# antonbaumann/MIMO-Unet

Measured on AMD Instinct MI355X. Metric: train images/sec at 256x256, S=2, fbc=30, higher is better.
Workload: dtype f32 (split into 16-bit hi/lo pairs on the MFMA; weight gradient: activation as one fp16 value); 1 GPU; cfg3: SEN12TP-shape synthetic 2->1 ch, 256x256, S=2, fbc=30, laplace_nll, batch 32 global; global_batch=32, per_gpu_batch=32, scaling=strong, labels=U[0,1) (SURVEY 8d); same batch every step, parallelism=dp1, world_size=1, weak_per_gpu_batch=32, strong_global_batch=32, optimizer=adam(lr=1e-3) fused, inputs=resident in HBM

## Files before the change

### include/mimo_hip.h

```cpp
#ifndef MIMO_HIP_H
#define MIMO_HIP_H

#include <stddef.h>
#include <stdint.h>

#ifdef __cplusplus
extern "C" {
#endif
#if defined(__GNUC__) || defined(__clang__)
#pragma GCC visibility push(default)
#endif

typedef struct mimo_plan mimo_plan;
typedef void* mimo_stream;

enum mimo_status {
  MIMO_OK = 0,
  MIMO_ERR_INVALID = -1,
  MIMO_ERR_HIP = -2,
  MIMO_ERR_STATE = -3
};

enum mimo_precision {
  MIMO_PREC_FP32 = 0,
// ... 214 lines not shown
  const float* z;
  int32_t ldz;
  const float *scale, *shift, *mean, *invstd;
  const float* mask;
  float* dz;
  float *dgamma, *dbeta, *dbias;
  float *c1, *c2;
  float *head_dw, *head_db;
  float* absmax;
  int32_t absmax_capacity;
  int32_t* absmax_n;
  int32_t* status;
} mimo_op_bn_relu_backward_args;
int mimo_op_bn_relu_backward(const mimo_op_bn_relu_backward_args* args, mimo_stream stream);

typedef struct mimo_op_head_backward_args {
  const float* a;
  int32_t lda;
  const float* w;
  int32_t c, c_p, co, n, subnetworks, s;
  int64_t hw;
  const float *out, *dout, *dloss, *label, *mask;
  const int64_t* perm;
  int32_t loss_kind;
  float eps_min, eps_max;
  const float *in_scale, *in_shift;
  int32_t precision;
  float *da, *dw, *db;
} mimo_op_head_backward_args;
int mimo_op_head_backward(const mimo_op_head_backward_args* args, mimo_stream stream);
// ... 109 lines not shown
```

### mimo_unet_amd/_lib.py

```python
from __future__ import annotations

import ctypes as C
import os

import torch

_HERE = os.path.dirname(os.path.abspath(__file__))
LIB_PATH = os.environ.get("MIMO_HIP_LIB") or os.path.join(_HERE, "libmimo_hip.so")


class MimoHipError(RuntimeError):
    pass


class MimoConfig(C.Structure):
    _fields_ = [
        ("in_channels", C.c_int32), ("out_channels", C.c_int32), ("num_subnetworks", C.c_int32),
        ("filter_base_count", C.c_int32), ("batch", C.c_int32), ("height", C.c_int32), ("width", C.c_int32),
        ("encoder_dropout_rate", C.c_float), ("core_dropout_rate", C.c_float), ("decoder_dropout_rate", C.c_float),
        ("bn_eps", C.c_float), ("bn_momentum", C.c_float), ("loss_kind", C.c_int32),
        ("eps_min", C.c_float), ("eps_max", C.c_float), ("device", C.c_int32), ("precision", C.c_int32),
        ("inference_only", C.c_int32), ("center_dropout_rate", C.c_float), ("final_dropout_rate", C.c_float),
        ("norm_kind", C.c_int32), ("act_kind", C.c_int32), ("up_kind", C.c_int32),
    ]
# ... 145 lines not shown
    "mimo_eval_accumulate": (C.c_int, [_P, _P, _P, _P, _P, _I, _I, _I, _I, _L, _I, _F, _F, _P, _I, _P, _P, _P]),
    "mimo_eval_select": (C.c_int, [_P, _L, _P, _I, _P, _P]),
    "mimo_eval_interval_sums": (C.c_int, [_P, _L, _I, _I, _P, _P, _P]),
    "mimo_eval_accumulate_sources": (C.c_int, [_P, _P, _P, _P, _P, _I, _I, _I, _I, _L, _I, _F, _F, _P, _I, _P, _P, _P, _P]),
    "mimo_eval_select_by": (C.c_int, [_P, _I, _L, _P, _I, _P, _P]),
    "mimo_eval_interval_sums_by": (C.c_int, [_P, _I, _P, _I, _L, _I, _I, _P, _P, _P]),
    "mimo_op_conv3x3_forward": (C.c_int, [_P, _P, _P, _P, _P, _I, _I, _I, _I, _I, _I, _I, _I, _P]),
    "mimo_op_conv3x3_dgrad": (C.c_int, [_P, _P, _P, _I, _I, _I, _I, _I, _I, _I, _I, _P]),
    "mimo_op_conv3x3_wgrad": (C.c_int, [_P, _P, _P, _P, _I, _I, _I, _I, _I, _I, _I, _I, _P]),
    "mimo_op_maxpool2x2": (C.c_int, [_P, _P, _I, _I, _I, _I, _P]),
    "mimo_op_upsample_cat": (C.c_int, [_P, _P, _P, _I, _I, _I, _I, _I, _I, _I, _P]),
    "mimo_op_fold_slice": (C.c_int, [_P, _I, _I, _P, _I, _I, _I, _I, _I, _I, _I, _P]),
    "mimo_op_pool_backward": (C.c_int, [_P, _I, _I, _P, _I, _P, _I, _P, _I, _I, _I, _I, _I, _I, _I, _P]),
    "mimo_op_up_backward": (C.c_int, [_P, _I, _I, _P, _I, _I, _I, _I, _I, _I, _I, _I, _I, _P]),
    "mimo_op_bn_relu_backward": (C.c_int, [C.POINTER(BnReluBackwardArgs), _P]),
    "mimo_op_head_backward": (C.c_int, [C.POINTER(HeadBackwardArgs), _P]),
    "mimo_op_bn_stats": (C.c_int, [C.POINTER(BnStatsArgs), _P]),
    "mimo_op_bn_relu_forward": (C.c_int, [C.POINTER(BnReluForwardArgs), _P]),
    "mimo_op_maxpool2x2_ex": (C.c_int, [_P, _I, _P, _I, _I, _I, _I, _I, _I, _P]),
    "mimo_op_upsample_cat_ex": (C.c_int, [_P, _I, _P, _I, _P, _P, _P, _I, _I, _I, _I, _I, _I, _I, _I, _P]),
    "mimo_op_head_forward": (C.c_int, [C.POINTER(HeadForwardArgs), _P]),
    "mimo_op_loss_forward": (C.c_int, [_P, _P, _P, _P, _I, _I, _I, _I, _I, _F, _F, _P, _P]),
    "mimo_op_pack_input": (C.c_int, [_P, _L, _L, _L, _P, _I, _I, _I, _I, _I, _P, _I, _P]),
    "mimo_op_unpack_dx": (C.c_int, [_P, _I, _I, _I, _I, _I, _I, _I, _I, _P, _P]),
    "mimo_op_fold_image_grad": (C.c_int, [_P, _I, _I, _I, _I, _I, _P, _I, _P]),
    "mimo_op_fold_image_grad_mc": (C.c_int, [_P, _I, _I, _I, _I, _I, _I, _P, _I, _P]),
    "mimo_monitor_grid_shape": (C.c_int, [C.c_int, C.c_int, C.c_int, C.c_int, C.c_int, C.POINTER(C.c_int), C.POINTER(C.c_int)]),
    "mimo_monitor_scratch_bytes": (C.c_size_t, [C.c_int]),
    "mimo_monitor_grids": (C.c_int, [C.POINTER(MonitorPanel), C.c_int, _P, _P, _P]),
    "mimo_dataset_gather": (C.c_int, [C.POINTER(GatherField), C.c_int, _P, _P, _L, _I, _I, _I, _P]),
# ... 37 lines not shown
```

### mimo_unet_amd/csrc/conv_thin.hip

```cpp
#include <algorithm>

#include "common.h"

namespace mimo {

namespace {

__device__ __forceinline__ float4 ld4f(const float* p) { return *reinterpret_cast<const float4*>(p); }
__device__ __forceinline__ void st4f(float* p, float4 v) { *reinterpret_cast<float4*>(p) = v; }

struct ThinMap {
  int q, pl, QB, PPI;
  bool active;
};
__device__ __forceinline__ ThinMap thin_map(int Cv) {
  ThinMap t;
  t.QB = Cv;
  t.PPI = 256 / Cv;
  t.q = threadIdx.x % Cv;
  t.pl = threadIdx.x / Cv;
  t.active = t.pl < t.PPI;
  return t;
}

// ... 241 lines not shown
      __syncthreads();
      if (t.pl == 0) {
        float4 s = red[t.q];
        for (int j = 1; j < t.PPI; ++j) {
          const float4 o = red[j * t.QB + t.q];
          s.x += o.x;
          s.y += o.y;
          s.z += o.z;
          s.w += o.w;
        }
        st4f(out + ((size_t)tap * CIN + ci) * 4 * Cv + c0, s);
      }
    }
}

__global__ __launch_bounds__(256) void wgrad_thin_reduce_kernel(const float* __restrict__ partial, int blocks, int cin, int Cp,
                                                                int cout, float* __restrict__ dw) {
  __shared__ double red[256];
  const int tc = blockIdx.x;
  const int tap = tc / cin, ci = tc - tap * cin;
  const int lanes = 256 / Cp;
  const int c = threadIdx.x % Cp, l = threadIdx.x / Cp;
  double s = 0.0;
  if (l < lanes)
    for (int b = l; b < blocks; b += lanes) s += (double)partial[((size_t)b * 9 * cin + tc) * Cp + c];
  red[threadIdx.x] = s;
  __syncthreads();
  if (l == 0 && c < cout) {
    for (int j = 1; j < lanes; ++j) s += red[j * Cp + c];
    dw[((size_t)c * cin + ci) * 9 + tap] = (float)s;
// ... 7 lines not shown
bool thin_enabled() { return thin_level() != 0; }

}

constexpr int kThinBlocks = 2048;

template <typename K>
static int resident_blocks(K kernel) {
  int dev = 0, cus = 256, per_cu = 2;
  if (hipGetDevice(&dev) == hipSuccess) {
    (void)hipDeviceGetAttribute(&cus, hipDeviceAttributeMultiprocessorCount, dev);
    if (hipOccupancyMaxActiveBlocksPerMultiprocessor(&per_cu, kernel, 256, 0) != hipSuccess || per_cu < 1) per_cu = 2;
  }
  return std::min(cus * per_cu, kThinBlocks);
}
struct ThinCaps {
  int fwd[4], wg[4];
};
static const ThinCaps& thin_caps() {
  static const ThinCaps c = {{resident_blocks(conv3x3_thin_fwd_kernel<1>), resident_blocks(conv3x3_thin_fwd_kernel<2>),
                              resident_blocks(conv3x3_thin_fwd_kernel<3>), resident_blocks(conv3x3_thin_fwd_kernel<4>)},
                             {resident_blocks(wgrad_thin_kernel<1>), resident_blocks(wgrad_thin_kernel<2>),
                              resident_blocks(wgrad_thin_kernel<3>), resident_blocks(wgrad_thin_kernel<4>)}};
  return c;
}

int conv3x3_thin_ok(int cin, int cout_p) {
  if (!(thin_enabled() && sched::thin_geometry_ok(cin, cout_p))) return 0;
  (void)thin_caps();
  return 1;
}

int conv3x3_thin_launch(const ConvLaunch& a, int cin, int* rows, hipStream_t stream) {
  if (!conv3x3_thin_ok(cin, a.cout_store) || a.off != 1 || a.Hi != a.Ho || a.Wi != a.Wo || a.Hi < 2 || a.Wi < 2 || a.cin_p < cin ||
      a.ldx % 4 != 0 || a.ldy % 4 != 0 || (int64_t)a.N * a.Hi * a.Wi > INT32_MAX) {
    set_error("conv3x3_thin: bad geometry cin=%d cout=%d H=%d W=%d", cin, a.cout_store, a.Hi, a.Wi);
    return MIMO_ERR_INVALID;
  }
// ... 28 lines not shown
  const int Cv = cout_p / 4;
  const int tilesY = (H + kTH - 1) / kTH, tilesX = (W + kTW - 1) / kTW, numTiles = N * tilesY * tilesX;
  const int blocks = std::min(numTiles, thin_caps().wg[cin - 1]);
  switch (cin) {
    case 1: hipLaunchKernelGGL(wgrad_thin_kernel<1>, dim3(blocks), dim3(256), 0, stream, x, ldx, dz, lddz, N, H, W, Cv, tilesY, tilesX, numTiles, partial); break;
    case 2: hipLaunchKernelGGL(wgrad_thin_kernel<2>, dim3(blocks), dim3(256), 0, stream, x, ldx, dz, lddz, N, H, W, Cv, tilesY, tilesX, numTiles, partial); break;
    case 3: hipLaunchKernelGGL(wgrad_thin_kernel<3>, dim3(blocks), dim3(256), 0, stream, x, ldx, dz, lddz, N, H, W, Cv, tilesY, tilesX, numTiles, partial); break;
    default: hipLaunchKernelGGL(wgrad_thin_kernel<4>, dim3(blocks), dim3(256), 0, stream, x, ldx, dz, lddz, N, H, W, Cv, tilesY, tilesX, numTiles, partial); break;
  }
  MIMO_KERNEL_CHECK();
  hipLaunchKernelGGL(wgrad_thin_reduce_kernel, dim3(9 * cin), dim3(256), 0, stream, partial, blocks, cin, cout_p, cout, dw);
  MIMO_KERNEL_CHECK();
  return MIMO_OK;
}

}
```

### mimo_unet_amd/csrc/elementwise.h

```cpp
#pragma once
#include "common.h"

namespace mimo {

constexpr int kMaxChunks = 64;
constexpr int kEwMaxBlocks = 1024;
constexpr int kBnReduceMaxBlocks = 2048;
constexpr int kMaxHeadOut = 8;

int rowsum_launch(const float* partial, int rows, int cols, double* sums, int* chunks, hipStream_t s);
constexpr int kColsumMaxRows = 2048;
constexpr int kStatusFwdStats = 1, kStatusBwdStats = 2, kStatusLogits = 4;
int colsum_vec_launch(const float* partial, int rows, int cols, int C, float* out, hipStream_t st);
int bn_fwd_stats_launch(const float* partial, int rows, int cout_pad, int C, int Cp, int64_t count, const float* gamma,
                        const float* beta, float* running_mean, float* running_var, float momentum, float eps, float* mean,
                        float* invstd, float* scale, float* shift, int* status, hipStream_t st);
int bn_bwd_stats_launch(const float* partial, int rows, int C, int Cp, int64_t count, int training, float* c1, float* c2,
                        float* dgamma, float* dbeta, float* dbias_zero, int* status, hipStream_t st);
int head_bwd_stats_launch(const float* partial, int rows, int C, int Cp, int Co, float* dw, float* db, hipStream_t st);

int pack_input_launch(const float* x, int64_t stride_n, int64_t stride_s, const int64_t* perm, int s, int N, int C,
                      int H, int W, float* out, int cp, hipStream_t st);
int unpack_dx_launch(const void* dxpad, int dt, int ldp, int N, int S, int s, int C, int H, int W, float* dx, hipStream_t st);

// ... 89 lines not shown
  }
};
int bnrelu_bwd_reduce_launch(const BnReluLayer& L, const GradSrc& src, const float* mask, float* partial, int* rows,
                             hipStream_t st);
struct BnBwdApplyOut {
  const float *c1, *c2;
  void* dz;
  int split_out;
  float* partial;
  int* rows;
  float* absmax;
  int* absmax_n;
  hipEvent_t done;
};
int bn_bwd_apply_launch(const BnReluLayer& L, const GradSrc& src, const float* mask, const BnBwdApplyOut& out, hipStream_t st);
int split_pairs_launch(const float* src, float* dst, int64_t P, int Cp, hipStream_t st, float* absmax = nullptr,
                       int* absmax_n = nullptr);

int head_fwd_launch(const void* a, int dt, int lda, const float* w, const float* bias, int C, int Co, int N, int S, int s,
                    int HW, float* out, hipStream_t st, int* status = nullptr, const float* in_scale = nullptr,
                    const float* in_shift = nullptr);
int loss_fwd_launch(const float* out, const float* label, const float* mask, const int64_t* perm, int N, int S,
                    int Co, int HW, int kind, float eps_min, float eps_max, float* partial, int* blocks,
                    hipStream_t st);
int loss_finalize_launch(const float* partial, int S, int blocks, double count, float* loss_out, hipStream_t st);
int head_bwd_launch(const void* a, int dt, int lda, const float* w, int C, int Cp, int Co, int N, int S, int s, int HW,
                    const float* out, const float* dout, const float* dloss, const float* label, const float* mask,
                    const int64_t* perm, int kind, float eps_min, float eps_max, void* da, float* partial,
                    int* rows, hipStream_t st, const float* in_scale = nullptr, const float* in_shift = nullptr);

// ... 2 lines not shown
```

### mimo_unet_amd/csrc/ew_bn_bwd.hip

```cpp
#include "ew_device.h"

namespace mimo {

__device__ __forceinline__ float route_max(float g, float v00, float v01, float v10, float v11, int self) {
  int arg = 0;
  float m = v00;
  if (v01 > m) { m = v01; arg = 1; }
  if (v10 > m) { m = v10; arg = 2; }
  if (v11 > m) { m = v11; arg = 3; }
  return arg == self ? g : 0.f;
}

template <typename T>
__global__ void pool_bwd_kernel(const T* __restrict__ dxpad, int ldp, int choff, const T* __restrict__ a,
                                int lda, T* __restrict__ da, int ldda, int N, int H, int W, int Cv, int accumulate,
                                const T* __restrict__ skip, int ldsk) {
  const PQ t = pixquad(Cv);
  if (!t.active) return;
  const int Hp = H / 2, Wp = W / 2;
  const int P = N * Hp * Wp;
  PixIter it = pix_iter(t.p, t.pstep, Hp, Wp);
  for (int p = t.p; p < P; p += t.pstep, pix_next(it, Hp, Wp)) {
    const int n = it.n, py = it.y, px = it.x;
    const float4 g = fold_read(dxpad, ldp, n, py, px, Hp, Wp, choff + 4 * t.q);
// ... 182 lines not shown
    st4(dst, v);
  }
}


int up_bwd_launch(const void* dxpad, int dt, int ldp, int choff, void* da, int ldda, int N, int H, int W, int h, int w,
                  int Cp, int accumulate, hipStream_t st) {
  const int Cv = Cp / 4;
  const int padT = (H - 2 * h) / 2, padL = (W - 2 * w) / 2;
  MIMO_ST_DISPATCH(dt, T, hipLaunchKernelGGL(up_bwd_kernel<T>, pq_grid(Cv, (int64_t)N * h * w, kBlocksUpBwd), dim3(256), 0, st,
                                             (const T*)dxpad, ldp, choff, (T*)da, ldda, N, H, W, h, w, padT, padL, Cv, accumulate));
  MIMO_KERNEL_CHECK();
  return MIMO_OK;
}

__device__ __forceinline__ float4 relu_gate4(float4 g, float4 v, float4 sc, float4 sh) {
  g.x = fmaf(v.x, sc.x, sh.x) > 0.f ? g.x : 0.f;
  g.y = fmaf(v.y, sc.y, sh.y) > 0.f ? g.y : 0.f;
  g.z = fmaf(v.z, sc.z, sh.z) > 0.f ? g.z : 0.f;
  g.w = fmaf(v.w, sc.w, sh.w) > 0.f ? g.w : 0.f;
  return g;
}

template <typename TZ, typename TA>
__device__ __forceinline__ int pool_cell4(const GradSrc& s, const TZ* z, int ldz, int n, int cy, int cx, int H, int W, int q,
                                          float4 sc, float4 sh, bool masked, float4 m, float4 zz[4], float4 g[4]) {
  const int Hp = H / 2, Wp = W / 2, y0 = 2 * cy, x0 = 2 * cx;
  const bool win = cy < Hp && cx < Wp;
  const int valid = win ? 15 : ((1 | (x0 + 1 < W ? 2 : 0)) | (y0 + 1 < H ? (4 | (x0 + 1 < W ? 8 : 0)) : 0));
  const TZ* zs = z + (((size_t)n * H + y0) * W + x0) * ldz + 4 * q;
#pragma unroll
  for (int j = 0; j < 4; ++j) zz[j] = (valid >> j) & 1 ? ld4(zs + ((size_t)(j >> 1) * W + (j & 1)) * ldz) : f4zero();
  float4 gp = f4zero();
  if (win) gp = fold_read((const TA*)s.dxpad, s.ldp, n, cy, cx, Hp, Wp, s.choff + 4 * q);
#pragma unroll
  for (int j = 0; j < 4; ++j)
    g[j] = (s.skip && ((valid >> j) & 1)) ? fold_read((const TA*)s.skip, s.ldsk, n, y0 + (j >> 1), x0 + (j & 1), H, W, s.skoff + 4 * q)
                                           : f4zero();
// ... 6 lines not shown
      g[j].z = route_max(gp.z, act(zz[0].z, sc.z, sh.z, m.z), act(zz[1].z, sc.z, sh.z, m.z), act(zz[2].z, sc.z, sh.z, m.z), act(zz[3].z, sc.z, sh.z, m.z), j) + g[j].z;
      g[j].w = route_max(gp.w, act(zz[0].w, sc.w, sh.w, m.w), act(zz[1].w, sc.w, sh.w, m.w), act(zz[2].w, sc.w, sh.w, m.w), act(zz[3].w, sc.w, sh.w, m.w), j) + g[j].w;
    }
  }
#pragma unroll
  for (int j = 0; j < 4; ++j) {
    if (masked) {
      g[j].x *= m.x;
      g[j].y *= m.y;
      g[j].z *= m.z;
      g[j].w *= m.w;
    }
    g[j] = relu_gate4(g[j], zz[j], sc, sh);
  }
  return valid;
}

template <int SRC, typename TZ, typename TA>
__device__ __forceinline__ float4 relu_grad4(const GradSrc& s, const HeadLane& hl, const float* mask, int C, int p,
                                             const PixIter& it, int q, int H, int W, float4 v, float4 sc, float4 sh, float* d0,
                                             float* d1) {
  static_assert(SRC != GS_POOL, "pooled tensors: pool_cell4");
  float4 g;
  const int n = it.n;
  float4 m = make_float4(1.f, 1.f, 1.f, 1.f);
  if (mask) m = mask4(mask, n, C, 4 * q);
  if constexpr (SRC == GS_PLAIN) {
    g = ld4((const TA*)s.da + (size_t)p * s.ldda + 4 * q);
  } else if constexpr (SRC == GS_FOLD) {
    g = fold_read((const TA*)s.dxpad, s.ldp, n, it.y, it.x, H, W, 4 * q);
  } else {
    head_dlogit(s.head, hl, p, d0, d1);
    g = f4zero();
    g.x = fmaf(*d1, hl.w1.x, fmaf(*d0, hl.w0.x, g.x));
    g.y = fmaf(*d1, hl.w1.y, fmaf(*d0, hl.w0.y, g.y));
    g.z = fmaf(*d1, hl.w1.z, fmaf(*d0, hl.w0.z, g.z));
    g.w = fmaf(*d1, hl.w1.w, fmaf(*d0, hl.w0.w, g.w));
  }
  if (mask) {
    g.x *= m.x;
    g.y *= m.y;
    g.z *= m.z;
    g.w *= m.w;
  }
  return relu_gate4(g, v, sc, sh);
}

template <typename TZ, typename TA, int SRC>
__global__ __launch_bounds__(kBnReduceThreads) void bnrelu_bwd_reduce_kernel(
    const GradSrc src, const TZ* __restrict__ z, int ldz,
    const float* __restrict__ scale, const float* __restrict__ shift, const float* __restrict__ mean,
    const float* __restrict__ invstd, const float* __restrict__ mask, int C, int Cv, int N, int H, int W,
    float* __restrict__ partial) {
  __shared__ float4 red[kBnReduceThreads];
  const PQ t = pixquad<kBnReduceThreads>(Cv);
  const int Cp = 4 * Cv;
  float4 a1 = f4zero(), a2 = f4zero();
  float4 hw0 = f4zero(), hw1 = f4zero();
  float hb0 = 0.f, hb1 = 0.f;
  HeadLane hl = {};
// ... 194 lines not shown
                                    const float* __restrict__ invstd, const float* __restrict__ mask, int C,
                                    const float* __restrict__ c1, const float* __restrict__ c2, int Cv, int N, int H,
                                    int W, TA* __restrict__ dz, int split_out, float* __restrict__ partial,
                                    float* __restrict__ absmax) {
  __shared__ float4 red[256];
  const PQ t = pixquad(Cv);
  const int Cp = 4 * Cv;
  float4 acc = f4zero();
  float amax = 0.f;
  HeadLane hl = {};
  if constexpr (SRC == GS_HEAD) hl = head_lane(src.head, t.q, t.active);
  if (t.active) {
    const float4 sc = ld4(scale + 4 * t.q), sh = ld4(shift + 4 * t.q), mu = ld4(mean + 4 * t.q), is = ld4(invstd + 4 * t.q);
    const float4 k1 = ld4(c1 + 4 * t.q), k2 = ld4(c2 + 4 * t.q);
    auto emit = [&](int p, float4 g, float4 v) {
      float4 r;
      r.x = sc.x * (g.x - k1.x - (v.x - mu.x) * is.x * k2.x);
      r.y = sc.y * (g.y - k1.y - (v.y - mu.y) * is.y * k2.y);
      r.z = sc.z * (g.z - k1.z - (v.z - mu.z) * is.z * k2.z);
      r.w = sc.w * (g.w - k1.w - (v.w - mu.w) * is.w * k2.w);
      if (split_out)
        st_split4(reinterpret_cast<float*>(dz), p, Cp, t.q, r);
      else
        st4(dz + (size_t)p * Cp + 4 * t.q, r);
      acc = f4add(acc, r);
      amax = absmax4(amax, r);
    };
    if constexpr (SRC == GS_POOL) {
      const int Hc = (H + 1) / 2, Wc = (W + 1) / 2, P = N * Hc * Wc;
      PixIter it = pix_iter(t.p, t.pstep, Hc, Wc);
      for (int p = t.p; p < P; p += t.pstep, pix_next(it, Hc, Wc)) {
        float4 zz[4], g[4];
        const float4 m = mask ? mask4(mask, it.n, C, 4 * t.q) : make_float4(1.f, 1.f, 1.f, 1.f);
        const int valid = pool_cell4<TZ, TA>(src, z, ldz, it.n, it.y, it.x, H, W, t.q, sc, sh, mask != nullptr, m, zz, g);
        const int p0 = (it.n * H + 2 * it.y) * W + 2 * it.x;
// ... 58 lines not shown
```

### mimo_unet_amd/csrc/ew_device.h

```cpp
#pragma once
#include <hip/hip_ext.h>

#include <algorithm>
#include <cstdlib>

#include "elementwise.h"

namespace mimo {
namespace {

struct PQ {
  int q;
  int ql, pl;
  int QB, PPI;
  int p, pstep;
  bool active;
};

template <int T = 256>
__device__ __forceinline__ PQ pixquad(int Cv, bool xcd_bands = false) {
  PQ r;
  r.QB = Cv < T ? Cv : T;
  r.PPI = T / r.QB;
  r.ql = threadIdx.x % r.QB;
// ... 295 lines not shown
  const int64_t obase = (((int64_t)n * h.S + h.s) * 2) * h.HW + yx;
  float a = h.dout ? h.dout[obase] : 0.f, b = h.dout ? h.dout[obase + h.HW] : 0.f;
  if (h.dloss) {
    const int64_t src = h.perm ? h.perm[(int64_t)h.s * h.N + n] : n;
    const float mk = h.mask ? h.mask[src * h.HW + yx] : 1.f;
    const float mu = h.out[obase], lp = h.out[obase + h.HW], y = h.label[src * h.HW + yx];
    float gm, gl;
    nll_grad(h.kind, mu - y, lp, h.eps_min, h.eps_max, &gm, &gl);
    a += l.coef * mk * gm;
    b += l.coef * mk * gl;
  }
  *d0 = a;
  *d1 = b;
}

}
}
```

### mimo_unet_amd/csrc/ops_api.hip

```cpp
#include <algorithm>
#include <vector>

#include "elementwise.h"

using namespace mimo;
using pack::is_mixed;
using pack::store_type;

namespace {

struct Temp {
  const char* who;
  bool failed = false;
  std::vector<void*> ptrs;
  explicit Temp(const char* who_) : who(who_) {}
  ~Temp() {
    for (void* p : ptrs) (void)hipFree(p);
  }
  template <typename T>
  T* get(size_t count) {
    void* q = nullptr;
    if (hipMalloc(&q, std::max<size_t>(count, 1) * sizeof(T)) != hipSuccess) {
      failed = true;
      return nullptr;
// ... 433 lines not shown
  MIMO_TRY(bnrelu_bwd_reduce_launch(L, src, a.mask, partial, &rows, st));
  MIMO_TRY(bn_bwd_stats_launch(partial, rows, a.c, Cp, (int64_t)N * H * W, a.training ? 1 : 0, a.c1, a.c2, a.dgamma, a.dbeta,
                               a.training ? a.dbias : nullptr, status, st));
  if (a.kind == GS_HEAD) MIMO_TRY(head_bwd_stats_launch(head_partial, rows, a.c, Cp, 2, a.head_dw, a.head_db, st));
  int absmax_n = 0;
  MIMO_TRY(bn_bwd_apply_launch(L, src, a.mask, BnBwdApplyOut{a.c1, a.c2, dzs.out, a.split_out ? 1 : 0, a.training ? nullptr : partial,
                                                             &rows, a.absmax, &absmax_n, nullptr}, st));
  if (!a.training) MIMO_TRY(colsum_vec_launch(partial, rows, Cp, a.c, a.dbias, st));
  MIMO_TRY(stage_back(dzs, prec, st));
  MIMO_HIP_CHECK(hipStreamSynchronize(st));
  if (a.absmax_n) *a.absmax_n = absmax_n;
  if (a.status) MIMO_HIP_CHECK(hipMemcpy(a.status, status, sizeof(int), hipMemcpyDeviceToHost));
  return MIMO_OK;
}

int mimo_op_head_backward(const mimo_op_head_backward_args* p, mimo_stream stream) {
  hipStream_t st = (hipStream_t)stream;
  const char* who = "mimo_op_head_backward";
  if (!p) {
    set_error("%s: null arguments", who);
    return MIMO_ERR_INVALID;
  }
  const mimo_op_head_backward_args& a = *p;
  const int Cp = a.c_p;
  if (a.n < 1 || a.hw < 1 || (int64_t)a.n * a.hw >= (int64_t)1 << 31 || Cp < 8 || Cp % 8 != 0 || Cp > 256 || a.c < 1 || a.c > Cp ||
      bad_slice(who, "a", a.lda, 0, Cp) || a.co < 2 || a.co > kMaxHeadOut || (a.co & 1) || a.subnetworks < 1 || a.s < 0 ||
      a.s >= a.subnetworks || !a.a || !a.w || !a.da || !a.dw || !a.db || (!a.dout && !a.dloss) ||
      (a.dloss && (!a.out || !a.label)) || (!a.in_scale != !a.in_shift) ||
      (a.loss_kind != MIMO_LOSS_LAPLACE_NLL && a.loss_kind != MIMO_LOSS_GAUSSIAN_NLL)) {
    set_error("%s: unsupported geometry or a missing tensor (c_p a multiple of 8 up to 256, an even co <= %d, dout and / or dloss "
// ... 303 lines not shown
```

### mimo_unet_amd/csrc/plan.hip

```cpp
#include <algorithm>
#include <cstdarg>
#include <cstdio>
#include <cstdlib>
#include <cstring>
#include <memory>
#include <string>
#include <vector>

#include "dz_ring.h"
#include "elementwise.h"
#include "graph_replay.h"

namespace mimo {

static thread_local char g_error[512] = "";
void set_error(const char* fmt, ...) {
  va_list ap;
  va_start(ap, fmt);
  vsnprintf(g_error, sizeof(g_error), fmt, ap);
  va_end(ap);
}
const char* last_error() { return g_error; }

namespace {
// ... 284 lines not shown
        *s_partial = nullptr, *s_losspart = nullptr;
  float* s_headpart = nullptr;
  int head_rows = 0;
  double* s_sums = nullptr;
  int* d_status = nullptr;
  size_t cap_act = 0, cap_pad = 0, cap_slab = 0, cap_partial = 0, cap_sums = 0;
  float* s_kpart = nullptr;
  size_t cap_kpart = 0;

  bool wg_async = false;
  ConvEnv env;
  int wg_delay_us = 0;
  bool fuse_bwd_src = false;
  bool fuse_bn_in = true;
  bool fuse_bwd_pool = false, fuse_bwd_head = false;
  DzRing ring;
  hipEvent_t ev_stage = nullptr;
  bool any_mixed_dz = false;

  Profiler prof;
  int tier_of(int h) const {
    int t = 0, hh = H;
    while (t < Profiler::kTiers - 1 && hh > h) {
      hh /= 2;
      ++t;
    }
    return t;
  }

  bool graph_enabled = true;
// ... 124 lines not shown
    L.off_gamma = add_tensor(L.bn_name + ".weight", {L.Cout}, 0);
    L.off_beta = add_tensor(L.bn_name + ".bias", {L.Cout}, 0);
    L.off_rm = add_tensor(L.bn_name + ".running_mean", {L.Cout}, 1);
    L.off_rv = add_tensor(L.bn_name + ".running_var", {L.Cout}, 1);
  }

  int alloc_convbn(ConvBN& L, const std::vector<int>& in_chmap) {
    const ConvRecipe& r = L.r;
    const int n = L.N, h = L.H, w = L.W;
    const bool train_bufs = cfg.inference_only != 1;
    const bool wgrad_bufs = cfg.inference_only == 0;
    MIMO_TRY(dalloc(&L.wf, pack::image_elems(PK_F32, r.fwd.rows, L.cin_p)));
    if (train_bufs) MIMO_TRY(dalloc(&L.wd, pack::image_elems(PK_F32, r.dgrad.rows, L.cout_p)));
    MIMO_TRY(dalloc(&L.bias_p, r.fwd.rows));
    if (r.thin && wgrad_bufs) cap_slab = std::max(cap_slab, wgrad_thin_scratch(L.Cin, L.cout_p));
    if (r.wg_split && !r.dgrad.split) any_mixed_dz = true;
    cap_kpart = std::max(cap_kpart, std::max(r.fwd.kpart, r.dgrad.kpart));
    if (r.fwd.split && (cfg.precision == MIMO_PREC_SPLIT16 || cfg.precision == MIMO_PREC_FP16_MIXED)) {
      if (!wmax_pool) MIMO_TRY(dalloc(&wmax_pool, kMaxWmaxWords));
      if (wmax_used >= kMaxWmaxWords) {
        set_error("too many convolution layers (%d) for the fp16 weight-scale words", wmax_used + 1);
        return MIMO_ERR_INVALID;
      }
      L.wmax = wmax_pool + wmax_used++;
    }
    if (r.fwd.split) {
      uint16_t* q = nullptr;
      MIMO_TRY(dalloc(&q, pack::image_elems(pack::kind(cfg.precision, PACK_FWD, true, r.fwd.wide != 0),
                                            r.fwd.wide ? r.fwd.wide : r.fwd.rows, L.cin_p)));
      L.wf16 = q;
// ... 140 lines not shown
    if (cfg.inference_only != 0 && cfg.inference_only != 2) cfg.inference_only = 1;
    if (cfg.inference_only == 2 && cfg.precision != MIMO_PREC_FP32 && cfg.precision != MIMO_PREC_SPLIT16) {
      set_error("inference_only = 2 (input gradient only) exists for the fp32 and split16 precisions, not for precision %d", cfg.precision);
      return MIMO_ERR_INVALID;
    }
    mixed = pack::is_mixed(cfg.precision);
    f16 = cfg.precision == MIMO_PREC_FP16_MIXED;
    st = pack::store_type(cfg.precision);
    esz = store_bytes(st);
    {
      const int v = getenv("MIMO_FUSE_BWD_SRC") ? atoi(getenv("MIMO_FUSE_BWD_SRC")) : 1;
      fuse_bwd_src = !mixed && cfg.inference_only != 1 && v != 0;
      fuse_bwd_pool = fuse_bwd_src && v != 3;
      fuse_bwd_head = fuse_bwd_src && v != 2;
      fuse_bn_in = !(getenv("MIMO_FUSE_BN_IN") && atoi(getenv("MIMO_FUSE_BN_IN")) == 0);
    }
    if (cfg.precision < MIMO_PREC_FP32 || cfg.precision > MIMO_PREC_FP16_MIXED) {
      set_error("unknown precision %d", cfg.precision);
      return MIMO_ERR_INVALID;
    }
    if (cfg.norm_kind != MIMO_NORM_BATCH || cfg.act_kind != MIMO_ACT_RELU || cfg.up_kind != MIMO_UP_BILINEAR_ALIGN_CORNERS) {
      set_error("block variant norm %d / act %d / up %d is not implemented: only BatchNorm2d + ReLU + bilinear align_corners "
                "up-sampling, the reference's blocks (components.py:22-30, 77-85)", cfg.norm_kind, cfg.act_kind, cfg.up_kind);
      return MIMO_ERR_INVALID;
    }
    S = cfg.num_subnetworks;
    f = cfg.filter_base_count;
    N = cfg.batch;
    H = cfg.height;
    W = cfg.width;
// ... 143 lines not shown
          MIMO_HIP_CHECK(hipDeviceGetStreamPriorityRange(&least, &greatest));
          if (least != greatest)
            MIMO_HIP_CHECK(hipStreamCreateWithPriority(&ring.side, hipStreamNonBlocking, least));
          else
            MIMO_HIP_CHECK(hipStreamCreateWithFlags(&ring.side, hipStreamNonBlocking));
        }
        for (int i = 0; i < DzRing::kSlots; ++i)
          for (hipEvent_t* e : {&ring.ev_dz[i], &ring.ev_wg[i]}) MIMO_HIP_CHECK(hipEventCreateWithFlags(e, hipEventDisableTiming));
        MIMO_HIP_CHECK(hipEventCreateWithFlags(&ring.ev_join, hipEventDisableTiming));
        MIMO_HIP_CHECK(hipEventCreateWithFlags(&ev_stage, hipEventDisableTiming));
      }
    }
    MIMO_TRY(alloc_act(&s_dxpadA, cap_pad, st));
    MIMO_TRY(alloc_act(&s_dxpadB, cap_pad, st));
    MIMO_TRY(dalloc(&s_wslab, cap_slab));
    if (cap_kpart) MIMO_TRY(dalloc(&s_kpart, cap_kpart));
    MIMO_TRY(dalloc(&s_partial, cap_partial));
    if (fuse_bwd_src && !cfg.inference_only) MIMO_TRY(dalloc(&s_headpart, (size_t)kBnReduceMaxBlocks * (2 * pad_channels(f) + 2)));
    MIMO_TRY(dalloc(&s_sums, cap_sums));
    MIMO_TRY(dalloc(&s_losspart, (size_t)S * 512));
    MIMO_TRY(dalloc(&d_status, 1));
    {
      std::vector<PackJob> jobs, dg;
      for (auto& dc : dcs)
        for (ConvBN* L : {&dc->c1, &dc->c2}) {
          const ConvDir &fw = L->r.fwd, &dg_ = L->r.dgrad;
          jobs.push_back(pack::make_job(PACK_FWD, cfg.precision, fw.split, L->Cout, L->Cin, L->cin_p, L->cout_p, fw.rows, fw.wide, fw.pair,
                                        L->fwd_row_map, L->cin_map, fw.split ? L->wf16 : (void*)L->wf, L->wmax, L->off_w, L->off_b, L->bias_p));
          dg.push_back(pack::make_job(PACK_DGRAD, cfg.precision, dg_.split, L->Cout, L->Cin, L->cin_p, L->cout_p, dg_.rows, dg_.wide, dg_.pair,
                                      L->dg_row_map, L->dg_col_map, dg_.split ? L->wd16 : (void*)L->wd, nullptr, L->off_w));
// ... 455 lines not shown
    if (wg_delay_us > 0) MIMO_TRY(debug_delay_launch(wg_delay_us, ws));
    const int pr = prof.begin(MIMO_PROF_CONV_WGRAD, ws);
    if (thin_wg)
      MIMO_TRY(wgrad_thin_launch(L.in, L.ld_in, o.dz_wg, L.cout_p, L.N, L.H, L.W, L.Cin, L.Cout, L.cout_p, s_wslab, grads + L.off_w, ws));
    else if (L.r.wg_split)
      MIMO_TRY(wgrad_split_launch(wg, ws));
    else
      MIMO_TRY(wgrad_launch(wg, ws));
    prof.end(pr, 18.0 * L.Cin * L.Cout * (double)P, 4.0 * (double)P * (L.Cin + L.Cout), ws);
    if (!thin_wg)
      MIMO_TRY(wgrad_reduce_launch(s_wslab, wg.splits, wg.cin_pad, wg.cout_pad, L.cin_map, L.cin_p, L.Cin, L.Cout,
                                   grads + L.off_w, ws, wg.dz_absmax, wg.dz_absmax_n, release));
    return MIMO_OK;
  }

  int convbn_backward(ConvBN& L, const GradSrc& src, const float* mask, bool need_dgrad, float* dxpad_out, const BwdCall& call,
                      hipStream_t st) {
    if (call.ig) return need_dgrad ? convbn_input_grad(L, src, mask, dxpad_out, st) : MIMO_OK;
    const bool thin_wg = L.r.wg_thin && !need_dgrad && wgrad_thin_ok(L.Cin, L.cout_p, L.N, L.H, L.W);
    DzRing::Slot s = ring.acquire(wg_async && !prof.on);
    MIMO_TRY(bn_backward(L, src, mask, s, fwd_training, thin_wg, st));
    if (need_dgrad) MIMO_TRY(dgrad_conv(L, ring.dz[s.b], dxpad_out, st));
    hipStream_t ws = st;
    MIMO_TRY(ring.reader_stream(s, st, &ws));
    const hipEvent_t release = ring.release_on_launch(s, capturing, thin_wg);
    MIMO_TRY(wgrad_issue(L, s, thin_wg, ws, release));
    return ring.released(s, release != nullptr);
  }

  int dc_backward(DoubleConv* dc, bool need_input_grad, const BwdCall& call, hipStream_t st, const GradSrc* head_src = nullptr) {
    const int blk = prof.begin(Profiler::kTierBase + 2 * tier_of(dc->c1.H) + 1, st);
    const int rc = dc_backward_impl(dc, need_input_grad, call, st, head_src);
    prof.end(blk, 0.0, 0.0, st);
    return rc;
// ... 531 lines not shown
```

Baseline: 1352 images/s.

## Fuse BN-backward apply into thin image-conv weight-gradient kernel

For the first (image-input) convolution, whose input has only a few channels, the BN/ReLU backward apply step is folded into the thin weight-gradient kernel. Each tile recomputes dz from z and the upstream gradient in registers and accumulates it straight into the 3x3 weight gradient, so the full-resolution dz tensor is never written and read back. This adds a dedicated slab buffer, an environment switch and a standalone op entry point. The cost is more register pressure and arithmetic per pixel in the fused kernel, and it gives up the async dz-ring overlap on that layer.

```diff
diff --git a/include/mimo_hip.h b/include/mimo_hip.h
--- a/include/mimo_hip.h
+++ b/include/mimo_hip.h
@@ -252,6 +252,9 @@
 } mimo_op_bn_relu_backward_args;
 int mimo_op_bn_relu_backward(const mimo_op_bn_relu_backward_args* args, mimo_stream stream);
 
+int mimo_op_image_conv_backward(const mimo_op_bn_relu_backward_args* args, const float* x, int32_t cin, int32_t cin_p, float* dw,
+                                int32_t fused, mimo_stream stream);
+
 typedef struct mimo_op_head_backward_args {
   const float* a;
   int32_t lda;
diff --git a/mimo_unet_amd/_lib.py b/mimo_unet_amd/_lib.py
--- a/mimo_unet_amd/_lib.py
+++ b/mimo_unet_amd/_lib.py
@@ -183,6 +183,7 @@
     "mimo_op_pool_backward": (C.c_int, [_P, _I, _I, _P, _I, _P, _I, _P, _I, _I, _I, _I, _I, _I, _I, _P]),
     "mimo_op_up_backward": (C.c_int, [_P, _I, _I, _P, _I, _I, _I, _I, _I, _I, _I, _I, _I, _P]),
     "mimo_op_bn_relu_backward": (C.c_int, [C.POINTER(BnReluBackwardArgs), _P]),
+    "mimo_op_image_conv_backward": (C.c_int, [C.POINTER(BnReluBackwardArgs), _P, _I, _I, _P, _I, _P]),
     "mimo_op_head_backward": (C.c_int, [C.POINTER(HeadBackwardArgs), _P]),
     "mimo_op_bn_stats": (C.c_int, [C.POINTER(BnStatsArgs), _P]),
     "mimo_op_bn_relu_forward": (C.c_int, [C.POINTER(BnReluForwardArgs), _P]),
diff --git a/mimo_unet_amd/csrc/conv_thin.hip b/mimo_unet_amd/csrc/conv_thin.hip
--- a/mimo_unet_amd/csrc/conv_thin.hip
+++ b/mimo_unet_amd/csrc/conv_thin.hip
@@ -1,6 +1,7 @@
 #include <algorithm>
 
 #include "common.h"
+#include "ew_device.h"
 
 namespace mimo {
 
@@ -279,6 +280,105 @@
     }
 }
 
+template <int CIN, int SRC, int KG>
+__global__ __launch_bounds__(256, CIN <= 2 ? 3 : 1) void bn_bwd_apply_wgrad_thin_kernel(const GradSrc src, const float* __restrict__ z, int ldz,
+                                                                      const float* __restrict__ scale, const float* __restrict__ shift,
+                                                                      const float* __restrict__ mean, const float* __restrict__ invstd,
+                                                                      const float* __restrict__ mask, int C, const float* __restrict__ c1,
+                                                                      const float* __restrict__ c2, const float* __restrict__ x, int ldx,
+                                                                      int N, int H, int W, int Cv, int tilesY, int tilesX, int numTiles,
+                                                                      float* __restrict__ partial) {
+  static_assert(SRC == GS_PLAIN || SRC == GS_FOLD, "the image convolution's gradient sources");
+  constexpr int CP = Px<CIN>::N;
+  __shared__ __attribute__((aligned(16))) float xs[2][kHaloPix * CP];
+  __shared__ float4 red[256];
+  const ThinMap t = thin_map(Cv);
+  const int c0 = 4 * t.q;
+  float4 acc[9][CIN];
+#pragma unroll
+  for (int tap = 0; tap < 9; ++tap)
+#pragma unroll
+    for (int ci = 0; ci < CIN; ++ci) acc[tap][ci] = make_float4(0.f, 0.f, 0.f, 0.f);
+  float4 sc = f4zero(), sh = sc, mu = sc, is = sc, k1 = sc, k2 = sc;
+  if (t.active) {
+    sc = ld4f(scale + c0), sh = ld4f(shift + c0), mu = ld4f(mean + c0), is = ld4f(invstd + c0);
+    k1 = ld4f(c1 + c0), k2 = ld4f(c2 + c0);
+  }
+  const HeadLane hl = {};
+  Px<CIN> pre[kHaloPerThread];
+  int tile = blockIdx.x, buf = 0;
+  if (tile < numTiles) {
+    halo_load<CIN>(x, ldx, H, W, thin_tile(numTiles - 1 - tile, tilesY, tilesX), pre);
+    halo_store<CIN>(xs[0], pre);
+  }
+  __syncthreads();
+  for (; tile < numTiles; tile += gridDim.x, buf ^= 1) {
+    const ThinTile tt = thin_tile(numTiles - 1 - tile, tilesY, tilesX);
+    const int next = tile + gridDim.x;
+    if (next < numTiles) halo_load<CIN>(x, ldx, H, W, thin_tile(numTiles - 1 - next, tilesY, tilesX), pre);
+    const float* xb = xs[buf];
+    if (t.active)
+      for (int i0 = t.pl; i0 < kTH * kTW; i0 += KG * t.PPI) {
+        float4 g[KG];
+#pragma unroll
+        for (int u = 0; u < KG; ++u) {
+          const int i = i0 + u * t.PPI, ic = min(i, kTH * kTW - 1), r = ic / kTW, c = ic - r * kTW;
+          const int oy = tt.y0 + r, ox = tt.x0 + c;
+          PixIter it = {};
+          it.n = tt.n;
+          it.y = min(oy, H - 1);
+          it.x = min(ox, W - 1);
+          const int p = (tt.n * H + it.y) * W + it.x;
+          const float4 v = ld4f(z + (size_t)p * ldz + c0);
+          float d0, d1;
+          const float4 dy = relu_grad4<SRC, float, float>(src, hl, mask, C, p, it, t.q, H, W, v, sc, sh, &d0, &d1);
+          const float4 dzv = bn_bwd_dz4(dy, v, sc, mu, is, k1, k2);
+          g[u] = (i < kTH * kTW && oy < H && ox < W) ? dzv : make_float4(0.f, 0.f, 0.f, 0.f);
+        }
+#pragma unroll
+        for (int u = 0; u < KG; ++u) {
+          const int i = min(i0 + u * t.PPI, kTH * kTW - 1), r = i / kTW, c = i - r * kTW;
+#pragma unroll
+          for (int kh = 0; kh < 3; ++kh)
+#pragma unroll
+            for (int kw = 0; kw < 3; ++kw) {
+              const Px<CIN> xv = load_px<CIN>(xb + ((r + kh) * kHaloW + c + kw) * CP);
+#pragma unroll
+              for (int ci = 0; ci < CIN; ++ci) {
+                float4& d = acc[kh * 3 + kw][ci];
+                d.x = fmaf(xv.v[ci], g[u].x, d.x);
+                d.y = fmaf(xv.v[ci], g[u].y, d.y);
+                d.z = fmaf(xv.v[ci], g[u].z, d.z);
+                d.w = fmaf(xv.v[ci], g[u].w, d.w);
+              }
+            }
+        }
+      }
+    if (next < numTiles) halo_store<CIN>(xs[buf ^ 1], pre);
+    __syncthreads();
+  }
+  float* out = partial + (size_t)blockIdx.x * 9 * CIN * 4 * Cv;
+#pragma unroll
+  for (int tap = 0; tap < 9; ++tap)
+#pragma unroll
+    for (int ci = 0; ci < CIN; ++ci) {
+      __syncthreads();
+      red[threadIdx.x] = acc[tap][ci];
+      __syncthreads();
+      if (t.pl == 0) {
+        float4 s = red[t.q];
+        for (int j = 1; j < t.PPI; ++j) {
+          const float4 o = red[j * t.QB + t.q];
+          s.x += o.x;
+          s.y += o.y;
+          s.z += o.z;
+          s.w += o.w;
+        }
+        st4f(out + ((size_t)tap * CIN + ci) * 4 * Cv + c0, s);
+      }
+    }
+}
+
 __global__ __launch_bounds__(256) void wgrad_thin_reduce_kernel(const float* __restrict__ partial, int blocks, int cin, int Cp,
                                                                 int cout, float* __restrict__ dw) {
   __shared__ double red[256];
@@ -316,14 +416,23 @@
   }
   return std::min(cus * per_cu, kThinBlocks);
 }
+constexpr int kFusedKG(int cin) { return cin <= 2 ? 2 : 1; }
 struct ThinCaps {
   int fwd[4], wg[4];
+  int fused[2][4];
 };
 static const ThinCaps& thin_caps() {
   static const ThinCaps c = {{resident_blocks(conv3x3_thin_fwd_kernel<1>), resident_blocks(conv3x3_thin_fwd_kernel<2>),
                               resident_blocks(conv3x3_thin_fwd_kernel<3>), resident_blocks(conv3x3_thin_fwd_kernel<4>)},
                              {resident_blocks(wgrad_thin_kernel<1>), resident_blocks(wgrad_thin_kernel<2>),
-                              resident_blocks(wgrad_thin_kernel<3>), resident_blocks(wgrad_thin_kernel<4>)}};
+                              resident_blocks(wgrad_thin_kernel<3>), resident_blocks(wgrad_thin_kernel<4>)},
+#define FUSED_CAPS(SRC)                                                                     \
+  {resident_blocks(bn_bwd_apply_wgrad_thin_kernel<1, SRC, kFusedKG(1)>),                   \
+   resident_blocks(bn_bwd_apply_wgrad_thin_kernel<2, SRC, kFusedKG(2)>),                   \
+   resident_blocks(bn_bwd_apply_wgrad_thin_kernel<3, SRC, kFusedKG(3)>),                   \
+   resident_blocks(bn_bwd_apply_wgrad_thin_kernel<4, SRC, kFusedKG(4)>)}
+                             {FUSED_CAPS(GS_PLAIN), FUSED_CAPS(GS_FOLD)}};
+#undef FUSED_CAPS
   return c;
 }
 
@@ -382,4 +491,40 @@
   return MIMO_OK;
 }
 
-}
+int bn_bwd_apply_wgrad_thin_launch(const BnReluLayer& L, const GradSrc& src, const float* mask, const float* c1, const float* c2,
+                                   const float* x, int ldx, int cin, int cout, float* partial, float* dw, hipStream_t stream) {
+  const int N = L.N, H = L.H, W = L.W;
+  if (!conv3x3_thin_ok(cin, L.Cp) || H < 2 || W < 2 || ldx % 4 != 0 || L.ldz % 4 != 0 || L.dtz != ST_F32 || L.dta != ST_F32 ||
+      (src.kind != GS_PLAIN && src.kind != GS_FOLD) || (src.kind == GS_PLAIN && src.ldda % 4 != 0) ||
+      (src.kind == GS_FOLD && src.ldp % 4 != 0) || cout < 1 || cout > L.Cp || (int64_t)N * (H + 2) * (W + 2) > INT32_MAX) {
+    set_error("bn_bwd_apply_wgrad_thin: cin=%d cout_p=%d H=%d W=%d source %d unsupported (fp32 storage, plain or folded source)", cin,
+              L.Cp, H, W, src.kind);
+    return MIMO_ERR_INVALID;
+  }
+  const int Cv = L.Cp / 4;
+  const int tilesY = (H + kTH - 1) / kTH, tilesX = (W + kTW - 1) / kTW, numTiles = N * tilesY * tilesX;
+  const int blocks = std::min(numTiles, thin_caps().fused[src.kind == GS_FOLD ? 1 : 0][cin - 1]);
+#define FUSED_LAUNCH(CIN, SRC)                                                                                                      \
+  hipLaunchKernelGGL((bn_bwd_apply_wgrad_thin_kernel<CIN, SRC, kFusedKG(CIN)>), dim3(blocks), dim3(256), 0, stream, src,            \
+                     (const float*)L.z, L.ldz, L.scale, L.shift, L.mean, L.invstd, mask, L.C, c1, c2, x, ldx, N, H, W, Cv, tilesY, \
+                     tilesX, numTiles, partial)
+#define FUSED_LAUNCH_SRC(CIN)      \
+  if (src.kind == GS_FOLD)         \
+    FUSED_LAUNCH(CIN, GS_FOLD);    \
+  else                             \
+    FUSED_LAUNCH(CIN, GS_PLAIN)
+  switch (cin) {
+    case 1: FUSED_LAUNCH_SRC(1); break;
+    case 2: FUSED_LAUNCH_SRC(2); break;
+    case 3: FUSED_LAUNCH_SRC(3); break;
+    default: FUSED_LAUNCH_SRC(4); break;
+  }
+#undef FUSED_LAUNCH_SRC
+#undef FUSED_LAUNCH
+  MIMO_KERNEL_CHECK();
+  hipLaunchKernelGGL(wgrad_thin_reduce_kernel, dim3(9 * cin), dim3(256), 0, stream, partial, blocks, cin, L.Cp, cout, dw);
+  MIMO_KERNEL_CHECK();
+  return MIMO_OK;
+}
+
+}
diff --git a/mimo_unet_amd/csrc/elementwise.h b/mimo_unet_amd/csrc/elementwise.h
--- a/mimo_unet_amd/csrc/elementwise.h
+++ b/mimo_unet_amd/csrc/elementwise.h
@@ -127,6 +127,8 @@
   hipEvent_t done;
 };
 int bn_bwd_apply_launch(const BnReluLayer& L, const GradSrc& src, const float* mask, const BnBwdApplyOut& out, hipStream_t st);
+int bn_bwd_apply_wgrad_thin_launch(const BnReluLayer& L, const GradSrc& src, const float* mask, const float* c1, const float* c2,
+                                   const float* x, int ldx, int cin, int cout, float* partial, float* dw, hipStream_t st);
 int split_pairs_launch(const float* src, float* dst, int64_t P, int Cp, hipStream_t st, float* absmax = nullptr,
                        int* absmax_n = nullptr);
 
diff --git a/mimo_unet_amd/csrc/ew_bn_bwd.hip b/mimo_unet_amd/csrc/ew_bn_bwd.hip
--- a/mimo_unet_amd/csrc/ew_bn_bwd.hip
+++ b/mimo_unet_amd/csrc/ew_bn_bwd.hip
@@ -220,14 +220,6 @@
   return MIMO_OK;
 }
 
-__device__ __forceinline__ float4 relu_gate4(float4 g, float4 v, float4 sc, float4 sh) {
-  g.x = fmaf(v.x, sc.x, sh.x) > 0.f ? g.x : 0.f;
-  g.y = fmaf(v.y, sc.y, sh.y) > 0.f ? g.y : 0.f;
-  g.z = fmaf(v.z, sc.z, sh.z) > 0.f ? g.z : 0.f;
-  g.w = fmaf(v.w, sc.w, sh.w) > 0.f ? g.w : 0.f;
-  return g;
-}
-
 template <typename TZ, typename TA>
 __device__ __forceinline__ int pool_cell4(const GradSrc& s, const TZ* z, int ldz, int n, int cy, int cx, int H, int W, int q,
                                           float4 sc, float4 sh, bool masked, float4 m, float4 zz[4], float4 g[4]) {
@@ -264,36 +256,6 @@
     g[j] = relu_gate4(g[j], zz[j], sc, sh);
   }
   return valid;
-}
-
-template <int SRC, typename TZ, typename TA>
-__device__ __forceinline__ float4 relu_grad4(const GradSrc& s, const HeadLane& hl, const float* mask, int C, int p,
-                                             const PixIter& it, int q, int H, int W, float4 v, float4 sc, float4 sh, float* d0,
-                                             float* d1) {
-  static_assert(SRC != GS_POOL, "pooled tensors: pool_cell4");
-  float4 g;
-  const int n = it.n;
-  float4 m = make_float4(1.f, 1.f, 1.f, 1.f);
-  if (mask) m = mask4(mask, n, C, 4 * q);
-  if constexpr (SRC == GS_PLAIN) {
-    g = ld4((const TA*)s.da + (size_t)p * s.ldda + 4 * q);
-  } else if constexpr (SRC == GS_FOLD) {
-    g = fold_read((const TA*)s.dxpad, s.ldp, n, it.y, it.x, H, W, 4 * q);
-  } else {
-    head_dlogit(s.head, hl, p, d0, d1);
-    g = f4zero();
-    g.x = fmaf(*d1, hl.w1.x, fmaf(*d0, hl.w0.x, g.x));
-    g.y = fmaf(*d1, hl.w1.y, fmaf(*d0, hl.w0.y, g.y));
-    g.z = fmaf(*d1, hl.w1.z, fmaf(*d0, hl.w0.z, g.z));
-    g.w = fmaf(*d1, hl.w1.w, fmaf(*d0, hl.w0.w, g.w));
-  }
-  if (mask) {
-    g.x *= m.x;
-    g.y *= m.y;
-    g.z *= m.z;
-    g.w *= m.w;
-  }
-  return relu_gate4(g, v, sc, sh);
 }
 
 template <typename TZ, typename TA, int SRC>
@@ -518,11 +480,7 @@
     const float4 sc = ld4(scale + 4 * t.q), sh = ld4(shift + 4 * t.q), mu = ld4(mean + 4 * t.q), is = ld4(invstd + 4 * t.q);
     const float4 k1 = ld4(c1 + 4 * t.q), k2 = ld4(c2 + 4 * t.q);
     auto emit = [&](int p, float4 g, float4 v) {
-      float4 r;
-      r.x = sc.x * (g.x - k1.x - (v.x - mu.x) * is.x * k2.x);
-      r.y = sc.y * (g.y - k1.y - (v.y - mu.y) * is.y * k2.y);
-      r.z = sc.z * (g.z - k1.z - (v.z - mu.z) * is.z * k2.z);
-      r.w = sc.w * (g.w - k1.w - (v.w - mu.w) * is.w * k2.w);
+      const float4 r = bn_bwd_dz4(g, v, sc, mu, is, k1, k2);
       if (split_out)
         st_split4(reinterpret_cast<float*>(dz), p, Cp, t.q, r);
       else
diff --git a/mimo_unet_amd/csrc/ew_device.h b/mimo_unet_amd/csrc/ew_device.h
--- a/mimo_unet_amd/csrc/ew_device.h
+++ b/mimo_unet_amd/csrc/ew_device.h
@@ -333,5 +333,52 @@
   *d1 = b;
 }
 
-}
-}
+__device__ __forceinline__ float4 relu_gate4(float4 g, float4 v, float4 sc, float4 sh) {
+  g.x = fmaf(v.x, sc.x, sh.x) > 0.f ? g.x : 0.f;
+  g.y = fmaf(v.y, sc.y, sh.y) > 0.f ? g.y : 0.f;
+  g.z = fmaf(v.z, sc.z, sh.z) > 0.f ? g.z : 0.f;
+  g.w = fmaf(v.w, sc.w, sh.w) > 0.f ? g.w : 0.f;
+  return g;
+}
+
+template <int SRC, typename TZ, typename TA>
+__device__ __forceinline__ float4 relu_grad4(const GradSrc& s, const HeadLane& hl, const float* mask, int C, int p,
+                                             const PixIter& it, int q, int H, int W, float4 v, float4 sc, float4 sh, float* d0,
+                                             float* d1) {
+  static_assert(SRC != GS_POOL, "pooled tensors: pool_cell4");
+  float4 g;
+  const int n = it.n;
+  float4 m = make_float4(1.f, 1.f, 1.f, 1.f);
+  if (mask) m = mask4(mask, n, C, 4 * q);
+  if constexpr (SRC == GS_PLAIN) {
+    g = ld4((const TA*)s.da + (size_t)p * s.ldda + 4 * q);
+  } else if constexpr (SRC == GS_FOLD) {
+    g = fold_read((const TA*)s.dxpad, s.ldp, n, it.y, it.x, H, W, 4 * q);
+  } else {
+    head_dlogit(s.head, hl, p, d0, d1);
+    g = f4zero();
+    g.x = fmaf(*d1, hl.w1.x, fmaf(*d0, hl.w0.x, g.x));
+    g.y = fmaf(*d1, hl.w1.y, fmaf(*d0, hl.w0.y, g.y));
+    g.z = fmaf(*d1, hl.w1.z, fmaf(*d0, hl.w0.z, g.z));
+    g.w = fmaf(*d1, hl.w1.w, fmaf(*d0, hl.w0.w, g.w));
+  }
+  if (mask) {
+    g.x *= m.x;
+    g.y *= m.y;
+    g.z *= m.z;
+    g.w *= m.w;
+  }
+  return relu_gate4(g, v, sc, sh);
+}
+
+__device__ __forceinline__ float4 bn_bwd_dz4(float4 g, float4 v, float4 sc, float4 mu, float4 is, float4 k1, float4 k2) {
+  float4 r;
+  r.x = sc.x * (g.x - k1.x - (v.x - mu.x) * is.x * k2.x);
+  r.y = sc.y * (g.y - k1.y - (v.y - mu.y) * is.y * k2.y);
+  r.z = sc.z * (g.z - k1.z - (v.z - mu.z) * is.z * k2.z);
+  r.w = sc.w * (g.w - k1.w - (v.w - mu.w) * is.w * k2.w);
+  return r;
+}
+
+}
+}
diff --git a/mimo_unet_amd/csrc/ops_api.hip b/mimo_unet_amd/csrc/ops_api.hip
--- a/mimo_unet_amd/csrc/ops_api.hip
+++ b/mimo_unet_amd/csrc/ops_api.hip
@@ -471,6 +471,59 @@
   return MIMO_OK;
 }
 
+int mimo_op_image_conv_backward(const mimo_op_bn_relu_backward_args* p, const float* x, int32_t cin, int32_t cin_p, float* dw,
+                                int32_t fused, mimo_stream stream) {
+  hipStream_t st = (hipStream_t)stream;
+  const char* who = "mimo_op_image_conv_backward";
+  if (!p) {
+    set_error("%s: null arguments", who);
+    return MIMO_ERR_INVALID;
+  }
+  const mimo_op_bn_relu_backward_args& a = *p;
+  const int Cp = a.c_p, N = a.n, H = a.h, W = a.w;
+  if (bad_dims(who, N, H, W, Cp) || bad_slice(who, "z", a.ldz, 0, Cp)) return MIMO_ERR_INVALID;
+  if ((a.kind != GS_PLAIN && a.kind != GS_FOLD) || !a.training || a.precision < MIMO_PREC_FP32 || a.precision > MIMO_PREC_BF16 || a.c < 1 || a.c > Cp || !a.z ||
+      !a.scale || !a.shift || !a.mean || !a.invstd || !a.c1 || !a.c2 || !x || !dw || cin < 1 || cin_p < cin || cin_p % 4 != 0 ||
+      !conv3x3_thin_ok(cin, Cp)) {
+    set_error("%s: training mode, fp32, a plain or folded source, 1..4 image channels in a pitch of 4 and every tensor but dz needed "
+              "(kind %d, cin %d of %d, c %d of %d)", who, a.kind, cin, cin_p, a.c, Cp);
+    return MIMO_ERR_INVALID;
+  }
+  GradSrc src;
+  src.kind = a.kind;
+  if (a.kind == GS_PLAIN) {
+    if (!a.da || bad_slice(who, "da", a.ldda, 0, Cp)) return MIMO_ERR_INVALID;
+    src.da = a.da;
+    src.ldda = a.ldda;
+  } else {
+    if (!a.dxpad || a.choff != 0 || bad_slice(who, "dxpad", a.ldp, 0, Cp)) {
+      set_error("%s: the folded source needs dxpad with choff 0 and a pitch of at least c_p", who);
+      return MIMO_ERR_INVALID;
+    }
+    src.dxpad = a.dxpad;
+    src.ldp = a.ldp;
+  }
+  Temp t(who);
+  float* partial = t.get<float>((size_t)kBnReduceMaxBlocks * 2 * Cp);
+  float* slab = t.get<float>(wgrad_thin_scratch(cin, Cp));
+  float* dz = (fused || a.dz) ? a.dz : t.get<float>((size_t)N * H * W * Cp);
+  int* status = t.get<int>(1);
+  MIMO_TRY(t.ok());
+  const BnReluLayer L = {a.z, ST_F32, a.ldz, ST_F32, a.scale, a.shift, a.mean, a.invstd, a.c, Cp, N, H, W};
+  int rows = 0;
+  MIMO_TRY(bnrelu_bwd_reduce_launch(L, src, a.mask, partial, &rows, st));
+  MIMO_TRY(bn_bwd_stats_launch(partial, rows, a.c, Cp, (int64_t)N * H * W, 1, a.c1, a.c2, a.dgamma, a.dbeta, a.dbias, status, st));
+  if (fused) {
+    MIMO_TRY(bn_bwd_apply_wgrad_thin_launch(L, src, a.mask, a.c1, a.c2, x, cin_p, cin, a.c, slab, dw, st));
+  } else {
+    MIMO_TRY(bn_bwd_apply_launch(L, src, a.mask, BnBwdApplyOut{a.c1, a.c2, dz, 0, nullptr, &rows, nullptr, nullptr, nullptr}, st));
+    MIMO_TRY(wgrad_thin_launch(x, cin_p, dz, Cp, N, H, W, cin, a.c, Cp, slab, dw, st));
+  }
+  MIMO_HIP_CHECK(hipStreamSynchronize(st));
+  if (a.status) MIMO_HIP_CHECK(hipMemcpy(a.status, status, sizeof(int), hipMemcpyDeviceToHost));
+  return MIMO_OK;
+}
+
 int mimo_op_head_backward(const mimo_op_head_backward_args* p, mimo_stream stream) {
   hipStream_t st = (hipStream_t)stream;
   const char* who = "mimo_op_head_backward";
diff --git a/mimo_unet_amd/csrc/plan.hip b/mimo_unet_amd/csrc/plan.hip
--- a/mimo_unet_amd/csrc/plan.hip
+++ b/mimo_unet_amd/csrc/plan.hip
@@ -322,6 +322,9 @@
   bool fuse_bwd_src = false;
   bool fuse_bn_in = true;
   bool fuse_bwd_pool = false, fuse_bwd_head = false;
+  bool fuse_image_bwd = true;
+  float* s_thinslab = nullptr;
+  size_t cap_thinslab = 0;
   DzRing ring;
   hipEvent_t ev_stage = nullptr;
   bool any_mixed_dz = false;
@@ -476,6 +479,7 @@
     if (train_bufs) MIMO_TRY(dalloc(&L.wd, pack::image_elems(PK_F32, r.dgrad.rows, L.cout_p)));
     MIMO_TRY(dalloc(&L.bias_p, r.fwd.rows));
     if (r.thin && wgrad_bufs) cap_slab = std::max(cap_slab, wgrad_thin_scratch(L.Cin, L.cout_p));
+    if (r.wg_thin && wgrad_bufs && fuse_image_bwd) cap_thinslab = std::max(cap_thinslab, wgrad_thin_scratch(L.Cin, L.cout_p));
     if (r.wg_split && !r.dgrad.split) any_mixed_dz = true;
     cap_kpart = std::max(cap_kpart, std::max(r.fwd.kpart, r.dgrad.kpart));
     if (r.fwd.split && (cfg.precision == MIMO_PREC_SPLIT16 || cfg.precision == MIMO_PREC_FP16_MIXED)) {
@@ -646,6 +650,7 @@
       fuse_bwd_pool = fuse_bwd_src && v != 3;
       fuse_bwd_head = fuse_bwd_src && v != 2;
       fuse_bn_in = !(getenv("MIMO_FUSE_BN_IN") && atoi(getenv("MIMO_FUSE_BN_IN")) == 0);
+      fuse_image_bwd = !mixed && cfg.inference_only == 0 && !(getenv("MIMO_FUSE_IMAGE_BWD") && atoi(getenv("MIMO_FUSE_IMAGE_BWD")) == 0);
     }
     if (cfg.precision < MIMO_PREC_FP32 || cfg.precision > MIMO_PREC_FP16_MIXED) {
       set_error("unknown precision %d", cfg.precision);
@@ -819,6 +824,7 @@
     MIMO_TRY(alloc_act(&s_dxpadA, cap_pad, st));
     MIMO_TRY(alloc_act(&s_dxpadB, cap_pad, st));
     MIMO_TRY(dalloc(&s_wslab, cap_slab));
+    if (cap_thinslab && !cfg.inference_only) MIMO_TRY(dalloc(&s_thinslab, cap_thinslab));
     if (cap_kpart) MIMO_TRY(dalloc(&s_kpart, cap_kpart));
     MIMO_TRY(dalloc(&s_partial, cap_partial));
     if (fuse_bwd_src && !cfg.inference_only) MIMO_TRY(dalloc(&s_headpart, (size_t)kBnReduceMaxBlocks * (2 * pad_channels(f) + 2)));
@@ -1304,10 +1310,25 @@
     return MIMO_OK;
   }
 
+  int image_conv_backward(ConvBN& L, const GradSrc& src, const float* mask, hipStream_t st) {
+    int rows = 0;
+    const int64_t P = (int64_t)L.N * L.H * L.W;
+    int pr = prof.begin(MIMO_PROF_BN_BWD_REDUCE, st);
+    MIMO_TRY(bnrelu_bwd_reduce_launch(L.bn, src, mask, s_partial, &rows, st));
+    prof.end(pr, 0.0, (4.0 + src_bytes(src)) * (double)P * L.cout_p, st);
+    MIMO_TRY(bn_bwd_stats_launch(s_partial, rows, L.Cout, L.cout_p, P, 1, L.c1, L.c2, grads + L.off_gamma, grads + L.off_beta,
+                                 grads + L.off_b, d_status, st));
+    pr = prof.begin(MIMO_PROF_CONV_WGRAD, st);
+    MIMO_TRY(bn_bwd_apply_wgrad_thin_launch(L.bn, src, mask, L.c1, L.c2, L.in, L.ld_in, L.Cin, L.Cout, s_thinslab, grads + L.off_w, st));
+    prof.end(pr, 18.0 * L.Cin * L.Cout * (double)P, (4.0 + src_bytes(src)) * (double)P * L.cout_p + 4.0 * (double)P * L.ld_in, st);
+    return MIMO_OK;
+  }
+
   int convbn_backward(ConvBN& L, const GradSrc& src, const float* mask, bool need_dgrad, float* dxpad_out, const BwdCall& call,
                       hipStream_t st) {
     if (call.ig) return need_dgrad ? convbn_input_grad(L, src, mask, dxpad_out, st) : MIMO_OK;
     const bool thin_wg = L.r.wg_thin && !need_dgrad && wgrad_thin_ok(L.Cin, L.cout_p, L.N, L.H, L.W);
+    if (thin_wg && fuse_image_bwd && fwd_training && src.kind <= GS_FOLD) return image_conv_backward(L, src, mask, st);
     DzRing::Slot s = ring.acquire(wg_async && !prof.on);
     MIMO_TRY(bn_backward(L, src, mask, s, fwd_training, thin_wg, st));
     if (need_dgrad) MIMO_TRY(dgrad_conv(L, ring.dz[s.b], dxpad_out, st));
```

After: 1358 images/s (median of 6 runs). No clear change (+0.5%).
